# Blaizzy/mlx-audio

Hardware: AMD Instinct MI355X
Metric: audio samples/sec + real-time factor, Kokoro-82M TTS (higher is better)
Workload: dtype bf16 weights x fp32 activations: vocoder convs = fp16 hi pass (v_mfma_f32_32x32x16_f16) + block-scaled FP4 (e2m1) lo pass (v_mfma_scale_f32_32x32x64_f8f6f4 cbsz / blgp 4, OCP MX: E8M0 scale per row x 32 channels / per output column), fp32 accumulate; front end bf16 hi+lo split; 1 GPU; Kokoro-82M bf16 TTS, tokens->waveform, canonical short sentence T=80 F=264 (6.6 s @ 24 kHz); utterances_per_gpu=64, global_batch=64, samples_per_utterance=158400, parallelism=utterance-dp1, precision_mode=6, wire=fp32

## Files before the change

mlx_audio_amd/csrc/conv_common.h:

```cpp
#pragma once
#include <stdlib.h>
#include <type_traits>
#include "common.h"

namespace mi355conv {

__device__ __forceinline__ void glds16(const void* gsrc, void* ldst) {
  __builtin_amdgcn_global_load_lds((const __attribute__((address_space(1))) void*)gsrc,
                                   (__attribute__((address_space(3))) void*)ldst, 16, 0, 0);
}

__device__ __forceinline__ float gelu_erf(float x) { return 0.5f * x * (1.0f + erff(x * 0.70710678118654752f)); }
__device__ __forceinline__ float gelu_tanh(float x) { return 0.5f * x * (1.0f + tanhf(0.7978845608028654f * (x + 0.044715f * x * x * x))); }

template <int PREC>
__device__ __forceinline__ f32x16 mfma16(const bf16x8 a, const bf16x8 b, const f32x16 c) {
  if constexpr (PREC >= 3)
    return __builtin_amdgcn_mfma_f32_32x32x16_f16(__builtin_bit_cast(f16x8, a), __builtin_bit_cast(f16x8, b), c, 0, 0, 0);
  else
    return __builtin_amdgcn_mfma_f32_32x32x16_bf16(a, b, c, 0, 0, 0);
}
template <int PREC>
constexpr int a_images() { return (PREC == 2 || PREC == 4) ? 2 : 1; }
template <int PREC>
// ... 36 lines not shown
    const float sn = __builtin_amdgcn_sinf(k.al_rev * u);
    u = fmaf(k.ial, sn * sn, u);
  }
  return u;
}

__device__ __forceinline__ void lds_barrier() {
  asm volatile("s_waitcnt lgkmcnt(0)" ::: "memory");
  __builtin_amdgcn_s_barrier();
  asm volatile("" ::: "memory");
}

template <int MF, int NF, int WM, int WN, int EPI, bool EXT = false, int MT = MF, int MO = 0>
__device__ __forceinline__ void conv_epilogue(const mi355_conv_gemm_args& a, f32x16 (&acc)[MT][NF], const int b, const int l0,
                                              const int n0, const int wm, const int wn, const int lane, const int len_out,
                                              const bool folded) {
  const int len_up = a.lens_up ? a.lens_up[b] : a.up_Lout;
  const int len_up_c = len_up > 0 ? len_up : 1;
  float* yb = a.y + (int64_t)b * a.y_bstride;
  const float* rb = (a.res && !folded) ? a.res + (int64_t)b * a.res_bstride : nullptr;
  const bool accum = a.accumulate && !folded;
  const bool want_stats = a.stats_partial != nullptr;
  float sK[NF], s1[NF], s2[NF];
  int scnt[NF];
  const bool want_ext = EXT && a.ext_partial != nullptr;
#pragma unroll
  for (int nf = 0; nf < NF; ++nf) { sK[nf] = 0.f; s1[nf] = 0.f; s2[nf] = 0.f; scnt[nf] = 0; }
#pragma unroll
  for (int mf = 0; mf < MF; ++mf)
#pragma unroll
    for (int nf = 0; nf < NF; ++nf) {
      const int n = n0 + wn * WN + nf * 32 + (lane & 31);
      const bool nok = n < a.Cout;
      const int ncl = nok ? n : a.Cout - 1;
      int ocol = ncl, rph = 0;
      if (a.up_s) { rph = ncl / a.up_cout; ocol = ncl - rph * a.up_cout; }
      const float bias = a.bias ? a.bias[ocol] : 0.f;
      const float cscale = a.post_colscale ? a.post_colscale[ocol] : 1.f;
#pragma unroll
      for (int h = 0; h < 2; ++h) {
        int orows[8];
        bool ok[8];
        float rv[8];
#pragma unroll
        for (int q = 0; q < 8; ++q) {
          const int r = h * 8 + q;
// ... 225 lines not shown
          }
        }
#pragma unroll
        for (int q = 0; q < 8; ++q) {
          const int r = h * 8 + q;
          const float v = ((acc[mf][nf][r] + bias) + rv[q]) * oscale;
          *(float*)(yw + (yoff + (uint32_t)(mf * 32 + (r & 3) + 8 * (r >> 2)) * ystep)) = v;
        }
        __builtin_amdgcn_sched_barrier(0);
      }
  }
}

}

int mi355_conv_ws4_launch(const mi355_conv_gemm_args& a, hipStream_t st, int feat, int bn = 128);
bool mi355_conv_ws4_eligible(const mi355_conv_gemm_args& a, bool vec);
```

mlx_audio_amd/csrc/conv_gemm.hip:

```cpp
#include "conv_common.h"

using namespace mi355conv;

namespace {

constexpr int kThreads = 256;

struct split_geom {
  int ksplit, cpz;
  int lo_slices;
};

template <int BM, int BN, int PREC, bool VEC, bool SPLIT = false>
__global__ __launch_bounds__(kThreads) void conv_gemm_kernel(const mi355_conv_gemm_args a, const split_geom sg) {
  constexpr int WM = BM / 2, WN = BN / 2, MF = WM / 32, NF = WN / 32;
  constexpr int BBYTES = (BN / 32) * 2048;
  extern __shared__ __attribute__((aligned(16))) char smem[];

  const int tid = threadIdx.x, lane = tid & 63, wave = tid >> 6;
  const int wm = wave >> 1, wn = wave & 1;
  const int b = SPLIT ? (int)blockIdx.z / sg.ksplit : (int)blockIdx.z, l0 = blockIdx.x * BM, n0 = blockIdx.y * BN;
  const int len_out = a.lens_out ? a.lens_out[b] : a.Lout;
  if (l0 >= len_out) return;
  const int len_in = a.lens_in ? a.lens_in[b] : a.Lin;
// ... 548 lines not shown
    MI355_REQUIRE(a.stats_bstride % 2 == 0 && ((uintptr_t)a.stats_partial) % 8 == 0, "conv_gemm: stats_partial must be 8-byte aligned");
  }
  int tile = a.tile;
  t_mx_lo_slices = 0;
  if (a.y_split) {
    MI355_REQUIRE(a.y_split == 2 || a.y_split == 4, "conv_gemm: y_split must be 0, 2 (bfloat16 hi | lo) or 4 (IEEE half hi | lo)");
    MI355_REQUIRE(!a.accumulate, "conv_gemm: y_split cannot accumulate into y (y holds split words)");
    a.split_ws = nullptr;
  }
  if (a.x_split) {
    MI355_REQUIRE(a.x_split == a.precision && (a.precision == 2 || a.precision == 4), "conv_gemm: x_split must equal the launch's precision, 2 or 4");
    MI355_REQUIRE(a.pre_act == MI355_ACT_NONE && !a.pre_scale && !a.pre_fq, "conv_gemm: a split input takes no prologue");
    MI355_REQUIRE(!a.ext_partial && mi355_conv_ws4_eligible(a, vec), "conv_gemm: x_split needs 16-byte aligned channels-last rows and a window of <= 192 rows "
                  "(the wave-specialised kernel)");
    static const int ws_feat_x = getenv("MI355_CONV_WS_FEAT") ? atoi(getenv("MI355_CONV_WS_FEAT")) : 0;
    const int rc = a.Cout <= 64 ? mi355_conv_ws4_launch(a, st, ws_feat_x & 3, 64) : mi355_conv_ws4_launch(a, st, tile % 10000000 == 6128128 ? ((tile / 10000000) % 10) : ws_feat_x);
    return rc;
  }
  if (a.ext_partial) {
    MI355_REQUIRE(conv_ext_supported(a), "conv_gemm: ext_partial needs a launch mi355_conv_gemm_ext_supported accepts (pre_fq, precision 2, plain store, K > 1)");
    MI355_REQUIRE(a.ext_bstride % 2 == 0 && ((uintptr_t)a.ext_partial) % 8 == 0, "conv_gemm: ext_partial must be 8-byte aligned");
    static const int ws_feat_e = getenv("MI355_CONV_WS_FEAT") ? atoi(getenv("MI355_CONV_WS_FEAT")) : 0;
    return mi355_conv_ws4_launch(a, st, ws_feat_e & 3, a.Cout <= 64 ? 64 : 128);
  }
  if (a.precision == 5 || a.precision == 6) {
    static const long ws_min5 = getenv("MI355_CONV_WS_MIN_TILES") ? atol(getenv("MI355_CONV_WS_MIN_TILES")) : 128;
    static const bool no_ws5 = getenv("MI355_CONV_NO_WS") != nullptr;
    const long wgs128 = (long)a.B * ((a.Lout + 127) / 128) * ((a.Cout + 127) / 128);
    const bool want = tile % 10000000 == 6128128 || (tile == 0 && !no_ws5 && a.Cout > 64 && wgs128 >= ws_min5 && a.Cin >= 64);
    if (want && mi355_conv_ws4_eligible(a, vec)) {
      const int rc = mi355_conv_ws4_launch(a, st, tile == 0 ? 0 : (((tile / 10000000) % 10) | ((tile / 100000000) << 4)));
      if (rc != MI355_ERR_UNSUPPORTED) return rc;
    }
    MI355_REQUIRE(tile % 10000000 != 6128128, "conv_gemm: precisions 5 / 6 on the wave-specialised tile needs K = 3 (mod 4), a plain / LeakyReLU / Snake prologue, "
                  "no epilogue activation beyond LeakyReLU and 16-B aligned channels-last rows");
    t_mx_lo_slices = (a.K + 1) >> 1;
    a.precision = 4;
  }
  const bool mx_image = t_mx_lo_slices != 0;
  if (tile == 0) {
    const int bn = a.Cout <= 64 ? 64 : 128;
    const long wgs128 = (long)a.B * ((a.Lout + 127) / 128) * ((a.Cout + bn - 1) / bn);
    const int bm = (bn == 128 && wgs128 >= 512) ? 128 : 64;
    tile = bm * 1000 + bn;
    static const bool no_ws = getenv("MI355_CONV_NO_WS") != nullptr;
    static const int ws_feat = getenv("MI355_CONV_WS_FEAT") ? atoi(getenv("MI355_CONV_WS_FEAT")) : 0;
// ... 13 lines not shown
      const int ks = split_groups(wgs64, (a.Cin + 31) >> 5, a.K, (long)a.B * a.Lout, a.Cout, a.split_ws_bytes, 0);
      if (ks) return bn == 128 ? launch_split_p<64, 128>(a, st, ks) : launch_split_p<64, 64>(a, st, ks);
    }
  }
  if (tile % 10000000 == 2064128 || tile % 10000000 == 2064064) {
    MI355_REQUIRE(vec && a.split_ws, "conv_gemm: the split-K tiles need the 16-B aligned channels-last input path and a workspace (split_ws)");
    const bool wide = tile % 10000000 == 2064128;
    const long wgs64 = (long)a.B * ((a.Lout + 63) / 64) * ((a.Cout + (wide ? 127 : 63)) / (wide ? 128 : 64));
    const int ks = split_groups(wgs64, (a.Cin + 31) >> 5, a.K, (long)a.B * a.Lout, a.Cout, a.split_ws_bytes, tile / 10000000 ? tile / 10000000 : -1);
    MI355_REQUIRE(ks >= 2, "conv_gemm: nothing to split (C_in %d, K %d, workspace %lld bytes)", a.Cin, a.K, (long long)a.split_ws_bytes);
    return wide ? launch_split_p<64, 128>(a, st, ks) : launch_split_p<64, 64>(a, st, ks);
  }
  if (tile % 10000000 == 6128064) {
    MI355_REQUIRE(!mx_image, "conv_gemm: MX images (precision 5) have no 128 x 64 wave-specialised tile");
    MI355_REQUIRE(mi355_conv_ws4_eligible(a, vec), "conv_gemm: the wave-specialised tile needs 16-B aligned channels-last input rows and a window of <= 192 rows");
    return mi355_conv_ws4_launch(a, st, (tile / 10000000) & 11, 64);
  }
  if (tile % 10000000 == 6128128) {
    MI355_REQUIRE(mi355_conv_ws4_eligible(a, vec), "conv_gemm: the wave-specialised tile needs 16-B aligned channels-last input rows and a window of <= 192 rows");
    return mi355_conv_ws4_launch(a, st, ((tile / 10000000) % 10) | ((tile / 100000000) << 4));
  }
  if (a.stats_partial) {
    MI355_REQUIRE(vec, "conv_gemm: fused statistics need the 16-B aligned channels-last input path");
    tile = 128128;
  }
  if (!vec) {
    if (a.precision == 3) return launch<64, 64, 3, false>(a, st);
    if (a.precision == 4) return launch<64, 64, 4, false>(a, st);
    a.precision = 2;
    return launch<64, 64, 2, false>(a, st);
  }
  if (a.precision == 2) {
    switch (tile) {
      case 128128: return launch<128, 128, 2, true>(a, st);
      case 64128: return launch<64, 128, 2, true>(a, st);
// ... 25 lines not shown
```

mlx_audio_amd/csrc/conv_ws4.h:

```cpp
#pragma once
#include "conv_common.h"

namespace mi355conv {

extern int g_ws4_resident;

constexpr int kWs4Threads = 512;

enum { P_NONE = 0, P_LEAKY = 1, P_SNAKE = 2, P_SNAKEBETA = 3, P_ELU = 4 };

struct ws4_geom {
  int tiles_per_item, P, NT, glog, fold;
  int nch;
  int keff;
  int tap_rows;
  int R;
  int gemm;
  int nslices;
  int bn;
  int feat;
  int total_ids;
  unsigned long long* dbg;
};

constexpr int kDbgSlots = 48;

struct tile_t { int b, l0, n0, len_out, len_in; };

__device__ __forceinline__ bool decode_tile(const mi355_conv_gemm_args& a, const ws4_geom& q, const int id, tile_t& t) {
  const int kq = id >> 3;
  const int ny = kq % q.NT;
  const int pg = kq / q.NT;
  const int glog = q.glog;
  const int p = (((((pg >> glog) << 3) + (id & 7)) << glog)) | (pg & ((1 << glog) - 1));
  if (p >= q.P) return false;
  t.b = p / q.tiles_per_item;
  t.l0 = (p - t.b * q.tiles_per_item) * 128;
  t.n0 = ny * q.bn;
  t.len_out = a.lens_out ? a.lens_out[t.b] : a.Lout;
  if (t.l0 >= t.len_out) return false;
  t.len_in = a.lens_in ? a.lens_in[t.b] : a.Lin;
  return true;
}
__device__ __forceinline__ int next_work(const mi355_conv_gemm_args& a, const ws4_geom& q, int id, tile_t& t) {
  for (id += (int)gridDim.x; id < q.total_ids; id += (int)gridDim.x)
    if (decode_tile(a, q, id, t)) return id;
  return -1;
}

template <int PREC, int PRE, int EPI, bool GEMM, bool DBG = false, int ABL = 0, int BN = 128, bool FQ = false, bool CW = true>
__global__ __launch_bounds__(kWs4Threads, 4) void conv_ws4_kernel(const mi355_conv_gemm_args a, const ws4_geom q) {
  static_assert(!FQ || (!GEMM && (PRE == P_NONE || PRE == P_LEAKY || PRE == P_SNAKE)), "quantising prologues: conv mode, none / LeakyReLU / Snake");
  constexpr int BM = 128;
  static_assert(BN == 128 || BN == 64, "tile columns");
  constexpr bool MXP = PREC == 5 || PREC == 6;
  constexpr bool FP4 = PREC == 6;
// ... 14 lines not shown
  tile_t t0;
  int id0 = (int)blockIdx.x - (int)gridDim.x;
  id0 = next_work(a, q, id0, t0);
  if (id0 < 0) return;

  if (wave >= 4) {
    const int ptid = tid - 256;
    const int c4 = (ptid & 7) * 4;
    const int prow = ptid >> 3;
    const float* xbase = a.x + a.x_off;
    const int wrow0 = (wave - 4) * 8;
    constexpr int cstride = GEMM ? 64 : 32;
    float4 s0[NLD], s1[NLD];
    constexpr int NKC = 2 + ((PRE == P_SNAKE || PRE == P_SNAKEBETA) ? 1 : 0) + (PRE == P_SNAKEBETA ? 1 : 0);
    float4 k0[NKC], k1[NKC];
    struct item_t { int id, ci, b, l0, len_in; };
    auto advance = [&](item_t& it) {
      if (it.ci + 1 < nch) { ++it.ci; return; }
      tile_t t;
      it.id = next_work(a, q, it.id, t);
      it.ci = 0; it.b = t.b; it.l0 = t.l0; it.len_in = t.len_in;
    };

    constexpr bool FASTW = !FQ && (MXP || GEMM || PRE == P_NONE || PRE == P_LEAKY);
    const bool fastw_off = !MXP && (q.feat & 2);
    auto interior_window = [&](const item_t& it) {
      if (fastw_off) return false;
      if constexpr (GEMM) return it.l0 + 128 <= it.len_in && it.l0 + 128 <= a.Lin && it.ci * 64 + 64 <= a.Cin;
      const int r0 = it.l0 - a.pad;
      return r0 >= 0 && r0 + R <= it.len_in && r0 + R <= a.Lin && it.ci * 32 + 32 <= a.Cin;
    };
    auto loadA = [&](float4 (&areg)[NLD], float4 (&kreg)[NKC], const item_t& it) {
      const int chunk = it.ci, l0 = it.l0;
      const float* xb = xbase + (int64_t)it.b * a.x_bstride;
      {
        const int c = chunk * cstride + c4;
        const float* const safe = (const float*)a.w;
        const bool aff = !GEMM && a.pre_scale != nullptr;
        kreg[0] = *(const float4*)(aff ? a.pre_scale + (int64_t)it.b * a.pre_ld + c : safe);
        kreg[1] = *(const float4*)(aff ? a.pre_shift + (int64_t)it.b * a.pre_ld + c : safe);
        if constexpr (PRE == P_SNAKE || PRE == P_SNAKEBETA) kreg[2] = *(const float4*)(a.pre_alpha + c);
        if constexpr (PRE == P_SNAKEBETA) kreg[3] = *(const float4*)(a.pre_inv_beta + c);
      }
      if (FASTW && interior_window(it)) {
        const char* wb = (const char*)(xb + (int64_t)(GEMM ? l0 : l0 - a.pad) * a.ldx + chunk * cstride);
        const uint32_t loff = ((uint32_t)prow * (uint32_t)a.ldx + (uint32_t)c4) * 4u;
        const size_t pstep = (size_t)a.ldx * 128u;
#pragma unroll
        for (int i = 0; i < NLD; ++i) {
          const int ii = (GEMM || wrow0 + i * 32 < R) ? i : 0;
          if constexpr (GEMM) areg[i] = *(const float4*)(wb + (ii & 3) * pstep + (ii >> 2) * 128 + loff);
          else areg[i] = *(const float4*)(wb + ii * pstep + loff);
        }
        return;
      }
#pragma unroll
      for (int i = 0; i < NLD; ++i) {
        const int ii = (GEMM || wrow0 + i * 32 < R) ? i : 0;
        int gl = GEMM ? l0 + prow + 32 * (ii & 3) : l0 - a.pad + prow + 32 * ii;
        int c = chunk * cstride + (GEMM ? 32 * (ii >> 2) : 0) + c4;
        gl = gl < 0 ? 0 : (gl >= a.Lin ? a.Lin - 1 : gl);
        if (c >= a.Cin) c = 0;
        areg[i] = *(const float4*)(xb + (int64_t)gl * a.ldx + c);
      }
    };
    auto convertA_body = [&](const float4 (&areg)[NLD], const float4 (&kreg)[NKC], const item_t& it, char* A_hi, auto mask_tag) {
      constexpr bool MASK = decltype(mask_tag)::value;
      const int chunk = it.ci, l0 = it.l0, b = it.b, len_in = it.len_in;
      char* A_lo = A_hi + ABYTES;
      const int c = chunk * cstride + c4;
      float sc[4] = {1.f, 1.f, 1.f, 1.f}, sh[4] = {0.f, 0.f, 0.f, 0.f}, al[4] = {1.f, 1.f, 1.f, 1.f}, ial[4] = {1.f, 1.f, 1.f, 1.f};
      if constexpr (!GEMM) {
        const bool aff = a.pre_scale != nullptr;
// ... 17 lines not shown
          al[j] *= 0.15915494309189535f;
        }
      }
      const float slope = a.pre_slope;
      const FakeQuant fq = FQ ? FakeQuant(-a.pre_fq[2 * b], a.pre_fq[2 * b + 1]) : FakeQuant(0.f, 0.f);
      fq_coef fk[4];
      if constexpr (FQ) {
#pragma unroll
        for (int j = 0; j < 4; ++j)
          fk[j] = fq_load_coef(a.pre_scale, a.pre_shift, (int64_t)b * a.pre_ld, PRE == P_SNAKE ? MI355_ACT_SNAKE : MI355_ACT_NONE, a.pre_alpha, c + j);
      }
      const bool chan[4] = {c < a.Cin, c + 1 < a.Cin, c + 2 < a.Cin, c + 3 < a.Cin};
      const bool xs = PRE == P_NONE && NA == 2 && !FQ && !MXP && a.x_split != 0;
#pragma unroll
      for (int i = 0; i < NLD; ++i) {
        if (GEMM || wrow0 + i * 32 < R) {
          const int r = prow + i * 32;
          if (GEMM || r < R) {
            const int gl = GEMM ? l0 + prow + 32 * (i & 3) : l0 - a.pad + r;
            const bool rowok = gl >= 0 && gl < len_in;
            const int cb = c + (GEMM ? 32 * (i >> 2) : 0);
            const float v[4] = {areg[i].x, areg[i].y, areg[i].z, areg[i].w};
            if constexpr (PRE == P_NONE && NA == 2 && !FQ && !MXP) {
              if (xs) {
                uint32_t w[4];
#pragma unroll
                for (int j = 0; j < 4; ++j) w[j] = (!MASK || (rowok && (cb + j) < a.Cin)) ? __builtin_bit_cast(uint32_t, v[j]) : 0u;
                const int xaddr = r * 64 + ((((c4 >> 3) ^ ((r >> 2) & 3))) << 4) + ((c4 & 4) << 1);
                uint2 xh, xl;
                xh.x = __builtin_amdgcn_perm(w[1], w[0], 0x05040100u);
                xh.y = __builtin_amdgcn_perm(w[3], w[2], 0x05040100u);
// ... 114 lines not shown
              if ((ptid & 7) == 0) *(uint8_t*)(A_l8 + R * LP + r) = (uint8_t)sb;
            }
          }
        }
      }
    };

    auto convertA = [&](const float4 (&areg)[NLD], const float4 (&kreg)[NKC], const item_t& it, char* A_hi) {
      if constexpr (FASTW) {
        if (interior_window(it)) { convertA_body(areg, kreg, it, A_hi, std::false_type{}); return; }
      }
      convertA_body(areg, kreg, it, A_hi, std::true_type{});
    };


    item_t ia{id0, 0, t0.b, t0.l0, t0.len_in};
    item_t ib = ia;
    advance(ib);
    constexpr bool work = (ABL & 4) == 0;
    unsigned long long* pdbg = nullptr;
    unsigned long long pc_conv = 0, pc_bar = 0, pc_load = 0, pc_items = 0, pc_first = 0, pc_t = 0;
    if constexpr (DBG && MXP) {
      if (wave == 4 && (blockIdx.x & 15) == 0 && q.dbg) pdbg = q.dbg + (size_t)(blockIdx.x >> 4) * kDbgSlots;
      if (pdbg) pc_first = pc_t = __builtin_amdgcn_s_memtime();
    }
    auto pstamp = [&](unsigned long long& acc_c) {
      if constexpr (DBG && MXP) {
        if (pdbg) { const unsigned long long n = __builtin_amdgcn_s_memtime(); acc_c += n - pc_t; pc_t = n; }
      }
    };
    if (work) loadA(s0, k0, ia);
// ... 40 lines not shown
  if (!(q.feat & 1)) __builtin_amdgcn_s_setprio(1);
  const int NTp = ((a.Cout + 127) >> 7) << 2;
  const int64_t wstep = (int64_t)NTp * 2048;
  const int nsteps = nch * keff;
  const int last_slice = q.nslices - 1;
  const int fold = q.fold;
  unsigned long long* dbg = nullptr;
  if constexpr (DBG) {
    if (wave == 0 && (blockIdx.x & 15) == 0 && q.dbg) dbg = q.dbg + (size_t)(blockIdx.x >> 4) * kDbgSlots;
  }
  int jbuf = 0;
  int ntile = 0;
  tile_t t = t0;
  for (int id = id0; id >= 0; id = next_work(a, q, id, t), ++ntile) {
    const int b = t.b, l0 = t.l0, n0 = t.n0, len_out = t.len_out;
    int lane = lane_k;
    asm volatile("" : "+v"(lane));
    const int hl = lane & 31, hh = lane >> 5;
    if constexpr (DBG) {
      if (dbg && lane == 0 && ntile < 8) dbg[4 * ntile] = __builtin_amdgcn_s_memtime();
      if (dbg && lane == 0 && (ntile == 0 || ntile == 7)) dbg[32 + (ntile == 7)] = wall_clock64();
    }
    const char* wfrag = (const char*)a.w + ((int64_t)((n0 >> 5) + wn * NF)) * 2048 + lane * 16;
    auto wptr = [&](const int s) { return wfrag + (int64_t)(s < last_slice ? s : last_slice) * wstep; };
    bf16x8 b0[NB], b1[NB];
    if constexpr (!MXP) {
#pragma unroll
      for (int f = 0; f < NB; ++f) b0[f] = *(const bf16x8*)(wfrag + f * 1024);
    }

// ... 25 lines not shown
#pragma unroll
            for (int r = 0; r < 16; ++r) rv[r] = *(const float*)(rw + (roff + (uint32_t)(mf * 32 + (r & 3) + 8 * (r >> 2)) * rpb + (uint32_t)(nf * 128)));
          }
          if (a.accumulate) {
#pragma unroll
            for (int r = 0; r < 16; ++r) rv[r] += *(const float*)(yr + (yoff + (uint32_t)(mf * 32 + (r & 3) + 8 * (r >> 2)) * ypb + (uint32_t)(nf * 128)));
          }
#pragma unroll
          for (int r = 0; r < 16; ++r) acc[mf][nf][r] = rv[r];
        }
    } else if ((ABL & 8) == 0 && fold) {
#pragma unroll
      for (int mf = 0; mf < MF; ++mf)
#pragma unroll
        for (int nf = 0; nf < NF; ++nf) {
          const int n = n0 + wn * WN + nf * 32 + hl;
          const bool nok = n < a.Cout;
          const int ncl = nok ? n : a.Cout - 1;
#pragma unroll
          for (int h = 0; h < 2; ++h) {
            float rv[8];
            int us[8];
#pragma unroll
            for (int qq = 0; qq < 8; ++qq) {
              const int r = h * 8 + qq;
              us[qq] = l0 + wm * WM + mf * 32 + (r & 3) + 8 * (r >> 2) + 4 * hh;
              rv[qq] = 0.f;
            }
            if (rb) {
#pragma unroll
// ... 25 lines not shown
        if constexpr ((ABL & 1) != 0) {
          if (!first) { asm volatile("" : "+v"(w) : "s"(src)); return; }
        }
        const i32x4 lo4 = *(const i32x4*)(src + wlane);
        if (FP4 && lo_item) {
          w = __builtin_shufflevector(lo4, lo4, 0, 1, 2, 3, 4, 5, 6, 7);
          return;
        }
        const i32x4 hi4 = *(const i32x4*)(src + 1024 + wlane);
        w = __builtin_shufflevector(lo4, hi4, 0, 1, 2, 3, 4, 5, 6, 7);
      };
      i32x8 w0, w1;
      ldW(w0, 0, true);
      if constexpr ((ABL & 1) != 0) w1 = w0;
      i32x8 qv[4];
      int sv[4] = {0, 0, 0, 0};
#pragma unroll
      for (int g = 0; g < 4; ++g)
#pragma unroll
        for (int e = 0; e < 8; ++e) qv[g][e] = 0;
      int hlx = hl, hhx = hh;
      int lbH = 0, lbL = 0, lbS = 0;
      auto fresh = [&]() {
        asm volatile("" : "+v"(hlx), "+v"(hhx));
        lbH = hlx * HP + hhx * 16;
        if constexpr (FP4) {
          lbL = (hlx + hhx * dil) * LP;
          lbS = hlx + hhx * dil;
        } else {
          lbL = hlx * LP + hhx * 16;
          lbS = hlx;
// ... 9 lines not shown
        i32x4 v0, v1;
        if constexpr ((ABL & 2) != 0) { v0 = (i32x4){la, la, la, la}; v1 = v0; }
        else {
          v0 = *(const i32x4*)(Abase + (la + uoff));
          v1 = *(const i32x4*)(Abase + (la + uoff) + 32 * HP);
        }
        qv[g] = __builtin_shufflevector(v0, v1, 0, 1, 2, 3, 4, 5, 6, 7);
      };
      auto rdL = [&](const int mf, const int p) {
        const int t1 = 2 * p + 1 < K ? 2 * p + 1 : K - 1;
        const int u0 = mf * 32 + 2 * p * dil, u1 = mf * 32 + t1 * dil;
        const int ubase = jbuf * WBYTES + ABYTES;
        int la = lbL, ls = lbS;
        asm volatile("" : "+v"(la), "+v"(ls));
        i32x4 x0, x1;
        int sc;
        if constexpr (FP4) {
          const int back = (2 * p + 1 < K) ? 0 : dil;
          if (back) { la -= hhx * back * LP; ls -= hhx * back; }
          x0 = *(const i32x4*)(Abase + (la + (ubase + u0 * LP)));
          x1 = x0;
          sc = (int)*(const uint8_t*)(Abase + (ls + (ubase + R * LP + u0)));
        } else if constexpr ((ABL & 2) != 0) {
          x0 = (i32x4){la, la, la, la}; x1 = x0; sc = 120 + (ls & 7);
        } else {
          x0 = *(const i32x4*)(Abase + (la + (ubase + u0 * LP)));
          x1 = *(const i32x4*)(Abase + (la + (ubase + u1 * LP)));
          sc = (int)*(const uint8_t*)(Abase + (ls + (ubase + R * LP + (hhx ? u1 : u0))));
        }
        qv[mf] = __builtin_shufflevector(x0, x1, 0, 1, 2, 3, 4, 5, 6, 7);
        sv[mf] = sc;
      };
      auto mmH = [&](const int g, const i32x8& w) {
        const int kk = g >> 1, m0 = 2 * (g & 1);
        const bf16x8 bfrag = kk ? hi4(w) : lo4(w);
        acc[m0][0] = mfma16<PREC>(lo4(qv[g]), bfrag, acc[m0][0]);
        acc[m0 + 1][0] = mfma16<PREC>(hi4(qv[g]), bfrag, acc[m0 + 1][0]);
      };
      auto mmL = [&](const int mf, const i32x8& w) {
        if constexpr (FP4) {
          const i32x4 a4 = __builtin_shufflevector(qv[mf], qv[mf], 0, 1, 2, 3), b4 = __builtin_shufflevector(w, w, 0, 1, 2, 3);
          asm volatile("s_nop 1\n\tv_mfma_scale_f32_32x32x64_f8f6f4 %0, %1, %2, %0, %3, %4 op_sel_hi:[0,0,0] cbsz:4 blgp:4" : "+v"(acc[mf][0]) : "v"(a4), "v"(b4), "v"(sv[mf]), "v"(bsc));
        } else {
          asm volatile("s_nop 1\n\tv_mfma_scale_f32_32x32x64_f8f6f4 %0, %1, %2, %0, %3, %4 op_sel_hi:[0,0,0]" : "+v"(acc[mf][0]) : "v"(qv[mf]), "v"(w), "v"(sv[mf]), "v"(bsc));
        }
      };
      auto hi_tap = [&](const int tp, const i32x8& w, auto last) {
        constexpr bool LAST = decltype(last)::value;
        fresh();
#pragma unroll
        for (int g = 0; g < 4; ++g) {
          mmH(g, w);
          if constexpr (LAST) rdL(g, 0);
          else rdH(g, tp + 1);
          __builtin_amdgcn_sched_barrier(0);
        }
      };
      auto lo_pair = [&](const int p, const i32x8& w, const bool more) {
        fresh();
// ... 136 lines not shown
        i32x4 x0, x1;
        int sc;
        if constexpr ((ABL & 2) != 0) {
          x0 = (i32x4){la, la, la, la}; x1 = x0; sc = 120 + (ls & 7);
        } else {
          x0 = *(const i32x4*)(Abase + (la + (ubase + u0 * LP)));
          x1 = *(const i32x4*)(Abase + (la + (ubase + u1 * LP)));
          sc = (int)*(const uint8_t*)(Abase + (ls + (ubase + R * LP + (hhx ? u1 : u0))));
        }
        if (mf == 0) { qa = __builtin_shufflevector(x0, x1, 0, 1, 2, 3, 4, 5, 6, 7); sa = sc; }
        else { qb = __builtin_shufflevector(x0, x1, 0, 1, 2, 3, 4, 5, 6, 7); sb2 = sc; }
      };
      auto mmH = [&](const int g, const i32x8 (&w)[2]) {
        const int kk = g >> 1, mf = g & 1;
        const bf16x8 h = g == 0 ? lo4(qa) : (g == 1 ? hi4(qa) : (g == 2 ? lo4(qb) : hi4(qb)));
#pragma unroll
        for (int nf = 0; nf < NF; ++nf) acc[mf][nf] = mfma16<PREC>(h, kk ? hi4(w[nf]) : lo4(w[nf]), acc[mf][nf]);
      };
      auto mmL = [&](const int mf, const i32x8 (&w)[2]) {
        if (mf == 0) {
          asm volatile("s_nop 1\n\tv_mfma_scale_f32_32x32x64_f8f6f4 %0, %1, %2, %0, %3, %4 op_sel_hi:[0,0,0]" : "+v"(acc[0][0]) : "v"(qa), "v"(w[0]), "v"(sa), "v"(bsc));
          asm volatile("v_mfma_scale_f32_32x32x64_f8f6f4 %0, %1, %2, %0, %3, %4 op_sel:[0,1,0] op_sel_hi:[0,0,0]" : "+v"(acc[0][1]) : "v"(qa), "v"(w[1]), "v"(sa), "v"(bsc));
        } else {
          asm volatile("s_nop 1\n\tv_mfma_scale_f32_32x32x64_f8f6f4 %0, %1, %2, %0, %3, %4 op_sel_hi:[0,0,0]" : "+v"(acc[1][0]) : "v"(qb), "v"(w[0]), "v"(sb2), "v"(bsc));
          asm volatile("v_mfma_scale_f32_32x32x64_f8f6f4 %0, %1, %2, %0, %3, %4 op_sel:[0,1,0] op_sel_hi:[0,0,0]" : "+v"(acc[1][1]) : "v"(qb), "v"(w[1]), "v"(sb2), "v"(bsc));
        }
      };
      auto hi_tap = [&](const int tp, const i32x8 (&w)[2], auto last) {
        constexpr bool LAST = decltype(last)::value;
        fresh();
        mmH(0, w);
        if constexpr (!LAST) rdH(0, tp + 1);
        __builtin_amdgcn_sched_barrier(0);
        mmH(1, w);
// ... 79 lines not shown
      auto rdA = [&](bf16x8& h, bf16x8& l, const int g, const int tp) {
        const int kk = g >> 1, mf = g & 1;
        const int row = wm * WM + mf * 32 + hl + tp * q.tap_rows;
        const int cidx = kk * 2 + hh;
        const int addr = row * 64 + ((cidx ^ ((row >> 2) & 3)) << 4);
        const char* A_hi = Abase + jbuf * WBYTES;
        if constexpr ((ABL & 2) != 0) {
          asm volatile("" : "+v"(h), "+v"(l) : "v"(addr));
        } else {
          h = *(const bf16x8*)(A_hi + addr);
          if constexpr (NA == 2) l = *(const bf16x8*)(A_hi + ABYTES + addr);
        }
      };
      auto mm = [&](const bf16x8& h, const bf16x8& l, const int g, const bf16x8 (&bf)[NB]) {
        const int kk = g >> 1, mf = g & 1;
#pragma unroll
        for (int nf = 0; nf < NF; ++nf) acc[mf][nf] = mfma16<PREC>(h, bf[2 * nf + kk], acc[mf][nf]);
        if constexpr (NA == 2) {
#pragma unroll
          for (int nf = 0; nf < NF; ++nf) acc[mf][nf] = mfma16<PREC>(l, bf[2 * nf + kk], acc[mf][nf]);
        }
      };
      auto tap_body = [&](const bf16x8 (&bf)[NB], const bool first) {
        if (tap == 0) {
          lds_barrier();
          if constexpr (DBG) {
            if (first && dbg && lane == 0 && ntile < 8) dbg[4 * ntile + 1] = __builtin_amdgcn_s_memtime();
          }
          rdA(ah0, al0, 0, 0);
        }
// ... 45 lines not shown
#pragma unroll
      for (int mf = 0; mf < MF; ++mf)
#pragma unroll
        for (int nf = 0; nf < NF; ++nf)
#pragma unroll
          for (int r = 0; r < 16; ++r) tsum += acc[mf][nf][r];
      if (tsum == 1.2345e-30f) yb[0] = tsum;
      continue;
    }
    const bool plain = a.up_s == 0 && a.post_act == MI355_ACT_NONE && (fold || (!a.res && !a.accumulate)) && !a.post_colscale && !a.y_split;
    if constexpr (COLW) {
      if (plain && interior) {
        conv_epilogue_interior<2, NF, 64, WN, FQ, MF, 0>(a, acc, b, l0, n0, 0, wn, lane);
        conv_epilogue_interior<2, NF, 64, WN, FQ, MF, 2>(a, acc, b, l0, n0, 1, wn, lane);
      } else {
        conv_epilogue<2, NF, 64, WN, EPI, FQ, MF, 0>(a, acc, b, l0, n0, 0, wn, lane, len_out, fold != 0);
        conv_epilogue<2, NF, 64, WN, EPI, FQ, MF, 2>(a, acc, b, l0, n0, 1, wn, lane, len_out, fold != 0);
      }
    } else {
      bool up_interior = false;
      if constexpr (EPI == 0 && !FQ && BN == 128 && PRE == P_LEAKY && !GEMM) {
        if (a.up_s != 0 && interior && a.post_act == MI355_ACT_NONE && !a.accumulate && !a.post_colscale && !a.y_split && !a.stats_partial && a.res_shift == 0 &&
            (a.up_cout & 31) == 0) {
          const int len_up = a.lens_up ? a.lens_up[b] : a.up_Lout;
          up_interior = (int64_t)l0 * a.up_s - a.up_p >= 0 && (int64_t)(l0 + BM - 1) * a.up_s + (a.up_s - 1) - a.up_p < len_up;
        }
      }
      if (plain && interior) conv_epilogue_interior<MF, NF, WM, WN, FQ>(a, acc, b, l0, n0, wm, wn, lane);
      else if (up_interior) conv_epilogue_up_interior<MF, NF, WM, WN>(a, acc, b, l0, n0, wm, wn, lane);
      else conv_epilogue<MF, NF, WM, WN, EPI, FQ>(a, acc, b, l0, n0, wm, wn, lane, len_out, fold != 0);
    }
    if constexpr (DBG) {
      if (dbg && lane == 0 && ntile < 8) dbg[4 * ntile + 3] = __builtin_amdgcn_s_memtime();
    }
  }
  if (!(q.feat & 1)) __builtin_amdgcn_s_setprio(0);
}

inline bool gemm_mode(const mi355_conv_gemm_args& a) { return a.K == 1 && a.Cin >= 64 && a.pre_act == MI355_ACT_NONE && !a.pre_scale && !a.pre_fq; }

template <int PREC, int PRE, int EPI, bool GEMM, bool DBG = false, int ABL = 0, int BN = 128, bool FQ = false, bool CW = true>
int launch_ws4(const mi355_conv_gemm_args& a, hipStream_t st, const int feat, unsigned long long* dbg = nullptr) {
  ws4_geom q;
  q.bn = BN;
  q.gemm = GEMM ? 1 : 0;
// ... 50 lines not shown
inline int pre_kind(const mi355_conv_gemm_args& a) {
  switch (a.pre_act) {
    case MI355_ACT_NONE: return P_NONE;
    case MI355_ACT_LEAKY: return P_LEAKY;
    case MI355_ACT_SNAKE: return a.pre_inv_beta ? P_SNAKEBETA : P_SNAKE;
    case MI355_ACT_ELU: return P_ELU;
  }
  return -1;
}

#define WS4_CASE(PREC, PRE, EPI) \
  if (bn == 128 && pre == PRE && epi == EPI && !gemm) return launch_ws4<PREC, PRE, EPI, false>(a, st, feat)
#define WS4_GEMM(PREC, EPI) \
  if (bn == 128 && epi == EPI && gemm) return launch_ws4<PREC, P_NONE, EPI, true>(a, st, feat)
#define WS4_CASE_N64(PREC, PRE, EPI) \
  if (bn == 64 && pre == PRE && epi == EPI && !gemm) return launch_ws4<PREC, PRE, EPI, false, false, 0, 64>(a, st, feat & 15)
#define WS4_GEMM_N64(PREC, EPI) \
  if (bn == 64 && epi == EPI && gemm) return launch_ws4<PREC, P_NONE, EPI, true, false, 0, 64>(a, st, feat & 15)

}

int mi355_conv_ws4_p2(const mi355_conv_gemm_args& a, hipStream_t st, int feat, unsigned long long* dbg, int bn);
int mi355_conv_ws4_p4(const mi355_conv_gemm_args& a, hipStream_t st, int feat, int bn);
int mi355_conv_ws4_p13(const mi355_conv_gemm_args& a, hipStream_t st, int feat, int bn);
int mi355_conv_ws4_fq(const mi355_conv_gemm_args& a, hipStream_t st, int feat, int bn);
int mi355_conv_ws4_p5(const mi355_conv_gemm_args& a, hipStream_t st, int feat, int bn);
int mi355_conv_ws4_p6(const mi355_conv_gemm_args& a, hipStream_t st, int feat, int bn);
int mi355_conv_ws4_p5_probe(const mi355_conv_gemm_args& a, hipStream_t st, int feat, unsigned long long* dbg);
```

mlx_audio_amd/csrc/conv_ws4.hip:

```cpp
#include "conv_ws4.h"

using namespace mi355conv;

namespace {
unsigned long long* g_dbg_buffer = nullptr;
}

namespace mi355conv {
int g_ws4_resident = 0;
}

extern "C" int mi355_conv_ws4_resident(int wgs) {
  MI355_REQUIRE(wgs >= 0, "conv_ws4_resident: negative count");
  mi355conv::g_ws4_resident = wgs;
  return MI355_OK;
}

bool mi355_conv_ws4_eligible(const mi355_conv_gemm_args& a, bool vec) {
  if (!vec || a.Lin <= 0 || a.flat_valid != 0) return false;
  if (a.precision == 5 || a.precision == 6)
    return a.K % 4 == 3 && 128 + (a.K - 1) * a.dil <= 192 && a.Cout > 64 && !a.pre_fq && (pre_kind(a) == P_NONE || pre_kind(a) == P_LEAKY || pre_kind(a) == P_SNAKE) &&
           epi_family(a) == 0;
  if (!gemm_mode(a) && 128 + (a.K - 1) * a.dil > 192) return false;
  return a.precision >= 1 && a.precision <= 4 && pre_kind(a) >= 0;
}

extern "C" int mi355_conv_ws4_debug_buffer(void* p) {
  g_dbg_buffer = (unsigned long long*)p;
  return MI355_OK;
}

int mi355_conv_ws4_p2(const mi355_conv_gemm_args& a, hipStream_t st, int feat, unsigned long long* dbg, int bn) {
  const int pre = pre_kind(a), epi = epi_family(a);
  const bool gemm = gemm_mode(a);
  if (bn == 128 && (feat & 4) && pre == P_SNAKE && epi == 0 && !gemm) return launch_ws4<2, P_SNAKE, 0, false, true>(a, st, feat, dbg);
  if (const int abl = bn == 128 ? feat >> 4 : 0) {
    if (gemm && epi == 0) {
      switch (abl) {
        case 1: return launch_ws4<2, P_NONE, 0, true, false, 1>(a, st, feat & 15);
        case 4: return launch_ws4<2, P_NONE, 0, true, false, 4>(a, st, feat & 15);
        case 5: return launch_ws4<2, P_NONE, 0, true, false, 5>(a, st, feat & 15);
      }
    }
    MI355_REQUIRE(pre == P_SNAKE && epi == 0 && !gemm, "conv_gemm(ws4): ablation tiles exist for the precision-2 Snake kernel and the plain GEMM mode only");
    switch (abl) {
      case 1: return launch_ws4<2, P_SNAKE, 0, false, false, 1>(a, st, feat & 15);
      case 2: return launch_ws4<2, P_SNAKE, 0, false, false, 2>(a, st, feat & 15);
      case 3: return launch_ws4<2, P_SNAKE, 0, false, false, 3>(a, st, feat & 15);
      case 4: return launch_ws4<2, P_SNAKE, 0, false, false, 4>(a, st, feat & 15);
      case 7: return launch_ws4<2, P_SNAKE, 0, false, false, 7>(a, st, feat & 15);
    }
// ... 8 lines not shown
  WS4_CASE(2, P_NONE, 1);
  WS4_GEMM(2, 0);
  WS4_GEMM(2, 1);
  WS4_GEMM(2, 2);
  WS4_GEMM(2, 3);
  WS4_CASE_N64(2, P_NONE, 0);
  WS4_CASE_N64(2, P_LEAKY, 0);
  WS4_CASE_N64(2, P_SNAKE, 0);
  WS4_CASE_N64(2, P_ELU, 0);
  WS4_GEMM_N64(2, 0);
  return MI355_ERR_UNSUPPORTED;
}

int mi355_conv_ws4_launch(const mi355_conv_gemm_args& a, hipStream_t st, int feat, int bn) {
  int rc = MI355_ERR_UNSUPPORTED;
  if (a.pre_fq) rc = a.precision == 2 ? mi355_conv_ws4_fq(a, st, feat & 3, bn) : MI355_ERR_UNSUPPORTED;
  else if (a.precision == 2) rc = mi355_conv_ws4_p2(a, st, feat, g_dbg_buffer, bn);
  else if (a.precision == 4) rc = mi355_conv_ws4_p4(a, st, feat & 3, bn);
  else if (a.precision == 6) rc = (feat & ~9) ? mi355_conv_ws4_p5_probe(a, st, feat, g_dbg_buffer) : mi355_conv_ws4_p6(a, st, feat & 9, bn);
  else if (a.precision == 5) rc = (feat & ~11) ? mi355_conv_ws4_p5_probe(a, st, feat, g_dbg_buffer) : mi355_conv_ws4_p5(a, st, feat & 11, bn);
  else if (a.precision == 1 || a.precision == 3) rc = mi355_conv_ws4_p13(a, st, feat & 3, bn);
  if (rc == MI355_ERR_UNSUPPORTED)
    mi355_set_error("conv_gemm(ws4): no instantiation for precision %d, prologue %d, epilogue family %d, %d-column tiles", a.precision, pre_kind(a), epi_family(a), bn);
  return rc;
}
```

mlx_audio_amd/csrc/conv_ws4_p5.hip:

```cpp
#include "conv_ws4.h"

using namespace mi355conv;

int mi355_conv_ws4_p5(const mi355_conv_gemm_args& a, hipStream_t st, int feat, int bn) {
  const int pre = pre_kind(a), epi = epi_family(a);
  const bool gemm = false;
  if ((feat & 2) && pre == P_SNAKE && epi == 0) return launch_ws4<5, P_SNAKE, 0, false, false, 0, 128, false, false>(a, st, feat & 9);
  WS4_CASE(5, P_NONE, 0);
  WS4_CASE(5, P_LEAKY, 0);
  WS4_CASE(5, P_SNAKE, 0);
  return MI355_ERR_UNSUPPORTED;
}
```

Before: 201.6 million samples/s.

## Skip dead 32-row blocks in tail tiles of wave-specialised conv kernel

Each tile now records how many of its four 32-row M blocks hold valid output rows, clamped by the sequence and upsampled lengths. The producer skips loads, the consumer skips the hi and lo MFMAs and epilogue stores for dead blocks, and fully dead waves only take part in the barriers. This removes wasted compute and memory traffic on partial tiles at the end of each utterance. Feature bit 128 turns the skip off, and the extra predicates and asm register pins add some branch and scheduling cost.

Result: slower. 197.8 million samples/s (-1.8%).

```diff
diff --git a/mlx_audio_amd/csrc/conv_common.h b/mlx_audio_amd/csrc/conv_common.h
--- a/mlx_audio_amd/csrc/conv_common.h
+++ b/mlx_audio_amd/csrc/conv_common.h
@@ -74,7 +74,7 @@
 template <int MF, int NF, int WM, int WN, int EPI, bool EXT = false, int MT = MF, int MO = 0>
 __device__ __forceinline__ void conv_epilogue(const mi355_conv_gemm_args& a, f32x16 (&acc)[MT][NF], const int b, const int l0,
                                               const int n0, const int wm, const int wn, const int lane, const int len_out,
-                                              const bool folded) {
+                                              const bool folded, const int mf_live = MF) {
   const int len_up = a.lens_up ? a.lens_up[b] : a.up_Lout;
   const int len_up_c = len_up > 0 ? len_up : 1;
   float* yb = a.y + (int64_t)b * a.y_bstride;
@@ -90,6 +90,7 @@
   for (int mf = 0; mf < MF; ++mf)
 #pragma unroll
     for (int nf = 0; nf < NF; ++nf) {
+      if (mf >= mf_live) continue;
       const int n = n0 + wn * WN + nf * 32 + (lane & 31);
       const bool nok = n < a.Cout;
       const int ncl = nok ? n : a.Cout - 1;
@@ -345,5 +346,7 @@
 
 }
 
+constexpr int kWs4FeatNoTailSkip = 128;
+inline int mi355_conv_ws4_tile_feat(const int tile) { return ((tile / 10000000) % 10) | ((tile / 100000000) << 4); }
 int mi355_conv_ws4_launch(const mi355_conv_gemm_args& a, hipStream_t st, int feat, int bn = 128);
 bool mi355_conv_ws4_eligible(const mi355_conv_gemm_args& a, bool vec);
diff --git a/mlx_audio_amd/csrc/conv_gemm.hip b/mlx_audio_amd/csrc/conv_gemm.hip
--- a/mlx_audio_amd/csrc/conv_gemm.hip
+++ b/mlx_audio_amd/csrc/conv_gemm.hip
@@ -586,7 +586,7 @@
     MI355_REQUIRE(!a.ext_partial && mi355_conv_ws4_eligible(a, vec), "conv_gemm: x_split needs 16-byte aligned channels-last rows and a window of <= 192 rows "
                   "(the wave-specialised kernel)");
     static const int ws_feat_x = getenv("MI355_CONV_WS_FEAT") ? atoi(getenv("MI355_CONV_WS_FEAT")) : 0;
-    const int rc = a.Cout <= 64 ? mi355_conv_ws4_launch(a, st, ws_feat_x & 3, 64) : mi355_conv_ws4_launch(a, st, tile % 10000000 == 6128128 ? ((tile / 10000000) % 10) : ws_feat_x);
+    const int rc = a.Cout <= 64 ? mi355_conv_ws4_launch(a, st, ws_feat_x & 3, 64) : mi355_conv_ws4_launch(a, st, tile % 10000000 == 6128128 ? (mi355_conv_ws4_tile_feat(tile) & (15 | kWs4FeatNoTailSkip)) : ws_feat_x);
     return rc;
   }
   if (a.ext_partial) {
@@ -601,7 +601,7 @@
     const long wgs128 = (long)a.B * ((a.Lout + 127) / 128) * ((a.Cout + 127) / 128);
     const bool want = tile % 10000000 == 6128128 || (tile == 0 && !no_ws5 && a.Cout > 64 && wgs128 >= ws_min5 && a.Cin >= 64);
     if (want && mi355_conv_ws4_eligible(a, vec)) {
-      const int rc = mi355_conv_ws4_launch(a, st, tile == 0 ? 0 : (((tile / 10000000) % 10) | ((tile / 100000000) << 4)));
+      const int rc = mi355_conv_ws4_launch(a, st, tile == 0 ? 0 : mi355_conv_ws4_tile_feat(tile));
       if (rc != MI355_ERR_UNSUPPORTED) return rc;
     }
     MI355_REQUIRE(tile % 10000000 != 6128128, "conv_gemm: precisions 5 / 6 on the wave-specialised tile needs K = 3 (mod 4), a plain / LeakyReLU / Snake prologue, "
@@ -645,11 +645,11 @@
   if (tile % 10000000 == 6128064) {
     MI355_REQUIRE(!mx_image, "conv_gemm: MX images (precision 5) have no 128 x 64 wave-specialised tile");
     MI355_REQUIRE(mi355_conv_ws4_eligible(a, vec), "conv_gemm: the wave-specialised tile needs 16-B aligned channels-last input rows and a window of <= 192 rows");
-    return mi355_conv_ws4_launch(a, st, (tile / 10000000) & 11, 64);
+    return mi355_conv_ws4_launch(a, st, mi355_conv_ws4_tile_feat(tile) & (11 | kWs4FeatNoTailSkip), 64);
   }
   if (tile % 10000000 == 6128128) {
     MI355_REQUIRE(mi355_conv_ws4_eligible(a, vec), "conv_gemm: the wave-specialised tile needs 16-B aligned channels-last input rows and a window of <= 192 rows");
-    return mi355_conv_ws4_launch(a, st, ((tile / 10000000) % 10) | ((tile / 100000000) << 4));
+    return mi355_conv_ws4_launch(a, st, mi355_conv_ws4_tile_feat(tile));
   }
   if (a.stats_partial) {
     MI355_REQUIRE(vec, "conv_gemm: fused statistics need the 16-B aligned channels-last input path");
diff --git a/mlx_audio_amd/csrc/conv_ws4.h b/mlx_audio_amd/csrc/conv_ws4.h
--- a/mlx_audio_amd/csrc/conv_ws4.h
+++ b/mlx_audio_amd/csrc/conv_ws4.h
@@ -25,7 +25,19 @@
 
 constexpr int kDbgSlots = 48;
 
-struct tile_t { int b, l0, n0, len_out, len_in; };
+struct tile_t { int b, l0, n0, len_out, len_in, mb; };
+
+__device__ __forceinline__ int tile_live_blocks(const mi355_conv_gemm_args& a, const ws4_geom& q, const tile_t& t) {
+  if (q.feat & kWs4FeatNoTailSkip) return 4;
+  int len = t.len_out;
+  if (a.up_s) {
+    const int len_up = a.lens_up ? a.lens_up[t.b] : a.up_Lout;
+    const int lu = (len_up + a.up_p + a.up_s - 1) / a.up_s;
+    len = lu < len ? lu : len;
+  }
+  const int mb = (len - t.l0 + 31) >> 5;
+  return mb < 1 ? 1 : (mb > 4 ? 4 : mb);
+}
 
 __device__ __forceinline__ bool decode_tile(const mi355_conv_gemm_args& a, const ws4_geom& q, const int id, tile_t& t) {
   const int kq = id >> 3;
@@ -40,6 +52,7 @@
   t.len_out = a.lens_out ? a.lens_out[t.b] : a.Lout;
   if (t.l0 >= t.len_out) return false;
   t.len_in = a.lens_in ? a.lens_in[t.b] : a.Lin;
+  t.mb = tile_live_blocks(a, q, t);
   return true;
 }
 __device__ __forceinline__ int next_work(const mi355_conv_gemm_args& a, const ws4_geom& q, int id, tile_t& t) {
@@ -84,12 +97,16 @@
     float4 s0[NLD], s1[NLD];
     constexpr int NKC = 2 + ((PRE == P_SNAKE || PRE == P_SNAKEBETA) ? 1 : 0) + (PRE == P_SNAKEBETA ? 1 : 0);
     float4 k0[NKC], k1[NKC];
-    struct item_t { int id, ci, b, l0, len_in; };
+    struct item_t { int id, ci, b, l0, len_in, mb; };
     auto advance = [&](item_t& it) {
       if (it.ci + 1 < nch) { ++it.ci; return; }
       tile_t t;
       it.id = next_work(a, q, it.id, t);
-      it.ci = 0; it.b = t.b; it.l0 = t.l0; it.len_in = t.len_in;
+      it.ci = 0; it.b = t.b; it.l0 = t.l0; it.len_in = t.len_in; it.mb = t.mb;
+    };
+    auto pass_live = [&](const int i, const item_t& it) {
+      if constexpr (GEMM) return (i & 3) < it.mb;
+      else return wrow0 + i * 32 < R - 32 * (4 - it.mb);
     };
 
     constexpr bool FASTW = !FQ && (MXP || GEMM || PRE == P_NONE || PRE == P_LEAKY);
@@ -118,7 +135,7 @@
         const size_t pstep = (size_t)a.ldx * 128u;
 #pragma unroll
         for (int i = 0; i < NLD; ++i) {
-          const int ii = (GEMM || wrow0 + i * 32 < R) ? i : 0;
+          const int ii = pass_live(i, it) ? i : 0;
           if constexpr (GEMM) areg[i] = *(const float4*)(wb + (ii & 3) * pstep + (ii >> 2) * 128 + loff);
           else areg[i] = *(const float4*)(wb + ii * pstep + loff);
         }
@@ -126,7 +143,7 @@
       }
 #pragma unroll
       for (int i = 0; i < NLD; ++i) {
-        const int ii = (GEMM || wrow0 + i * 32 < R) ? i : 0;
+        const int ii = pass_live(i, it) ? i : 0;
         int gl = GEMM ? l0 + prow + 32 * (ii & 3) : l0 - a.pad + prow + 32 * ii;
         int c = chunk * cstride + (GEMM ? 32 * (ii >> 2) : 0) + c4;
         gl = gl < 0 ? 0 : (gl >= a.Lin ? a.Lin - 1 : gl);
@@ -174,7 +191,7 @@
       const bool xs = PRE == P_NONE && NA == 2 && !FQ && !MXP && a.x_split != 0;
 #pragma unroll
       for (int i = 0; i < NLD; ++i) {
-        if (GEMM || wrow0 + i * 32 < R) {
+        if (pass_live(i, it)) {
           const int r = prow + i * 32;
           if (GEMM || r < R) {
             const int gl = GEMM ? l0 + prow + 32 * (i & 3) : l0 - a.pad + r;
@@ -319,7 +336,7 @@
     };
 
 
-    item_t ia{id0, 0, t0.b, t0.l0, t0.len_in};
+    item_t ia{id0, 0, t0.b, t0.l0, t0.len_in, t0.mb};
     item_t ib = ia;
     advance(ib);
     constexpr bool work = (ABL & 4) == 0;
@@ -390,6 +407,15 @@
   tile_t t = t0;
   for (int id = id0; id >= 0; id = next_work(a, q, id, t), ++ntile) {
     const int b = t.b, l0 = t.l0, n0 = t.n0, len_out = t.len_out;
+    const int mb = t.mb;
+    const int nlive = COLW ? mb : (mb - wm * MF < 0 ? 0 : (mb - wm * MF > MF ? MF : mb - wm * MF));
+    if constexpr (!COLW) {
+      if (nlive == 0) {
+        for (int c = 0; c < nch; ++c) lds_barrier();
+        jbuf ^= nch & 1;
+        continue;
+      }
+    }
     int lane = lane_k;
     asm volatile("" : "+v"(lane));
     const int hl = lane & 31, hh = lane >> 5;
@@ -445,6 +471,7 @@
       for (int mf = 0; mf < MF; ++mf)
 #pragma unroll
         for (int nf = 0; nf < NF; ++nf) {
+          if (mf >= nlive) continue;
           const int n = n0 + wn * WN + nf * 32 + hl;
           const bool nok = n < a.Cout;
           const int ncl = nok ? n : a.Cout - 1;
@@ -500,7 +527,7 @@
       ldW(w0, 0, true);
       if constexpr ((ABL & 1) != 0) w1 = w0;
       i32x8 qv[4];
-      int sv[4] = {0, 0, 0, 0};
+      uint8_t sv[4] = {0, 0, 0, 0};
 #pragma unroll
       for (int g = 0; g < 4; ++g)
 #pragma unroll
@@ -540,35 +567,44 @@
         int la = lbL, ls = lbS;
         asm volatile("" : "+v"(la), "+v"(ls));
         i32x4 x0, x1;
-        int sc;
+        uint8_t sc;
         if constexpr (FP4) {
           const int back = (2 * p + 1 < K) ? 0 : dil;
           if (back) { la -= hhx * back * LP; ls -= hhx * back; }
           x0 = *(const i32x4*)(Abase + (la + (ubase + u0 * LP)));
           x1 = x0;
-          sc = (int)*(const uint8_t*)(Abase + (ls + (ubase + R * LP + u0)));
+          sc = *(const uint8_t*)(Abase + (ls + (ubase + R * LP + u0)));
         } else if constexpr ((ABL & 2) != 0) {
           x0 = (i32x4){la, la, la, la}; x1 = x0; sc = 120 + (ls & 7);
         } else {
           x0 = *(const i32x4*)(Abase + (la + (ubase + u0 * LP)));
           x1 = *(const i32x4*)(Abase + (la + (ubase + u1 * LP)));
-          sc = (int)*(const uint8_t*)(Abase + (ls + (ubase + R * LP + (hhx ? u1 : u0))));
+          sc = *(const uint8_t*)(Abase + (ls + (ubase + R * LP + (hhx ? u1 : u0))));
         }
         qv[mf] = __builtin_shufflevector(x0, x1, 0, 1, 2, 3, 4, 5, 6, 7);
-        sv[mf] = sc;
+        sv[mf] = (uint8_t)sc;
       };
       auto mmH = [&](const int g, const i32x8& w) {
         const int kk = g >> 1, m0 = 2 * (g & 1);
         const bf16x8 bfrag = kk ? hi4(w) : lo4(w);
-        acc[m0][0] = mfma16<PREC>(lo4(qv[g]), bfrag, acc[m0][0]);
-        acc[m0 + 1][0] = mfma16<PREC>(hi4(qv[g]), bfrag, acc[m0 + 1][0]);
+        const bf16x8 a0 = lo4(qv[g]), a1 = hi4(qv[g]);
+        asm volatile("" ::"v"(a0));
+        if (m0 == 0 || m0 < mb) acc[m0][0] = mfma16<PREC>(a0, bfrag, acc[m0][0]);
+        asm volatile("" ::"v"(a1));
+        if (m0 + 1 < mb) acc[m0 + 1][0] = mfma16<PREC>(a1, bfrag, acc[m0 + 1][0]);
       };
       auto mmL = [&](const int mf, const i32x8& w) {
+        const bool dead = mf > 0 && mf >= mb;
+        const int sca = (int)sv[mf];
         if constexpr (FP4) {
           const i32x4 a4 = __builtin_shufflevector(qv[mf], qv[mf], 0, 1, 2, 3), b4 = __builtin_shufflevector(w, w, 0, 1, 2, 3);
-          asm volatile("s_nop 1\n\tv_mfma_scale_f32_32x32x64_f8f6f4 %0, %1, %2, %0, %3, %4 op_sel_hi:[0,0,0] cbsz:4 blgp:4" : "+v"(acc[mf][0]) : "v"(a4), "v"(b4), "v"(sv[mf]), "v"(bsc));
+          asm volatile("" ::"v"(a4), "v"(sca));
+          if (dead) return;
+          asm volatile("s_nop 1\n\tv_mfma_scale_f32_32x32x64_f8f6f4 %0, %1, %2, %0, %3, %4 op_sel_hi:[0,0,0] cbsz:4 blgp:4" : "+v"(acc[mf][0]) : "v"(a4), "v"(b4), "v"(sca), "v"(bsc));
         } else {
-          asm volatile("s_nop 1\n\tv_mfma_scale_f32_32x32x64_f8f6f4 %0, %1, %2, %0, %3, %4 op_sel_hi:[0,0,0]" : "+v"(acc[mf][0]) : "v"(qv[mf]), "v"(w), "v"(sv[mf]), "v"(bsc));
+          asm volatile("" ::"v"(qv[mf]), "v"(sca));
+          if (dead) return;
+          asm volatile("s_nop 1\n\tv_mfma_scale_f32_32x32x64_f8f6f4 %0, %1, %2, %0, %3, %4 op_sel_hi:[0,0,0]" : "+v"(acc[mf][0]) : "v"(qv[mf]), "v"(w), "v"(sca), "v"(bsc));
         }
       };
       auto hi_tap = [&](const int tp, const i32x8& w, auto last) {
@@ -735,10 +771,15 @@
       auto mmH = [&](const int g, const i32x8 (&w)[2]) {
         const int kk = g >> 1, mf = g & 1;
         const bf16x8 h = g == 0 ? lo4(qa) : (g == 1 ? hi4(qa) : (g == 2 ? lo4(qb) : hi4(qb)));
+        asm volatile("" ::"v"(h));
+        if (mf > 0 && mf >= nlive) return;
 #pragma unroll
         for (int nf = 0; nf < NF; ++nf) acc[mf][nf] = mfma16<PREC>(h, kk ? hi4(w[nf]) : lo4(w[nf]), acc[mf][nf]);
       };
       auto mmL = [&](const int mf, const i32x8 (&w)[2]) {
+        if (mf == 0) asm volatile("" ::"v"(qa), "v"(sa));
+        else asm volatile("" ::"v"(qb), "v"(sb2));
+        if (mf > 0 && mf >= nlive) return;
         if (mf == 0) {
           asm volatile("s_nop 1\n\tv_mfma_scale_f32_32x32x64_f8f6f4 %0, %1, %2, %0, %3, %4 op_sel_hi:[0,0,0]" : "+v"(acc[0][0]) : "v"(qa), "v"(w[0]), "v"(sa), "v"(bsc));
           asm volatile("v_mfma_scale_f32_32x32x64_f8f6f4 %0, %1, %2, %0, %3, %4 op_sel:[0,1,0] op_sel_hi:[0,0,0]" : "+v"(acc[0][1]) : "v"(qa), "v"(w[1]), "v"(sa), "v"(bsc));
@@ -848,6 +889,9 @@
       };
       auto mm = [&](const bf16x8& h, const bf16x8& l, const int g, const bf16x8 (&bf)[NB]) {
         const int kk = g >> 1, mf = g & 1;
+        if constexpr (NA == 2) asm volatile("" ::"v"(h), "v"(l));
+        else asm volatile("" ::"v"(h));
+        if (mf > 0 && mf >= nlive) return;
 #pragma unroll
         for (int nf = 0; nf < NF; ++nf) acc[mf][nf] = mfma16<PREC>(h, bf[2 * nf + kk], acc[mf][nf]);
         if constexpr (NA == 2) {
@@ -923,8 +967,8 @@
         conv_epilogue_interior<2, NF, 64, WN, FQ, MF, 0>(a, acc, b, l0, n0, 0, wn, lane);
         conv_epilogue_interior<2, NF, 64, WN, FQ, MF, 2>(a, acc, b, l0, n0, 1, wn, lane);
       } else {
-        conv_epilogue<2, NF, 64, WN, EPI, FQ, MF, 0>(a, acc, b, l0, n0, 0, wn, lane, len_out, fold != 0);
-        conv_epilogue<2, NF, 64, WN, EPI, FQ, MF, 2>(a, acc, b, l0, n0, 1, wn, lane, len_out, fold != 0);
+        conv_epilogue<2, NF, 64, WN, EPI, FQ, MF, 0>(a, acc, b, l0, n0, 0, wn, lane, len_out, fold != 0, mb);
+        if (mb > 2) conv_epilogue<2, NF, 64, WN, EPI, FQ, MF, 2>(a, acc, b, l0, n0, 1, wn, lane, len_out, fold != 0, mb - 2);
       }
     } else {
       bool up_interior = false;
@@ -937,7 +981,7 @@
       }
       if (plain && interior) conv_epilogue_interior<MF, NF, WM, WN, FQ>(a, acc, b, l0, n0, wm, wn, lane);
       else if (up_interior) conv_epilogue_up_interior<MF, NF, WM, WN>(a, acc, b, l0, n0, wm, wn, lane);
-      else conv_epilogue<MF, NF, WM, WN, EPI, FQ>(a, acc, b, l0, n0, wm, wn, lane, len_out, fold != 0);
+      else conv_epilogue<MF, NF, WM, WN, EPI, FQ>(a, acc, b, l0, n0, wm, wn, lane, len_out, fold != 0, nlive);
     }
     if constexpr (DBG) {
       if (dbg && lane == 0 && ntile < 8) dbg[4 * ntile + 3] = __builtin_amdgcn_s_memtime();
@@ -1018,9 +1062,9 @@
 #define WS4_GEMM(PREC, EPI) \
   if (bn == 128 && epi == EPI && gemm) return launch_ws4<PREC, P_NONE, EPI, true>(a, st, feat)
 #define WS4_CASE_N64(PREC, PRE, EPI) \
-  if (bn == 64 && pre == PRE && epi == EPI && !gemm) return launch_ws4<PREC, PRE, EPI, false, false, 0, 64>(a, st, feat & 15)
+  if (bn == 64 && pre == PRE && epi == EPI && !gemm) return launch_ws4<PREC, PRE, EPI, false, false, 0, 64>(a, st, feat & (15 | kWs4FeatNoTailSkip))
 #define WS4_GEMM_N64(PREC, EPI) \
-  if (bn == 64 && epi == EPI && gemm) return launch_ws4<PREC, P_NONE, EPI, true, false, 0, 64>(a, st, feat & 15)
+  if (bn == 64 && epi == EPI && gemm) return launch_ws4<PREC, P_NONE, EPI, true, false, 0, 64>(a, st, feat & (15 | kWs4FeatNoTailSkip))
 
 }
 
diff --git a/mlx_audio_amd/csrc/conv_ws4.hip b/mlx_audio_amd/csrc/conv_ws4.hip
--- a/mlx_audio_amd/csrc/conv_ws4.hip
+++ b/mlx_audio_amd/csrc/conv_ws4.hip
@@ -34,7 +34,7 @@
   const int pre = pre_kind(a), epi = epi_family(a);
   const bool gemm = gemm_mode(a);
   if (bn == 128 && (feat & 4) && pre == P_SNAKE && epi == 0 && !gemm) return launch_ws4<2, P_SNAKE, 0, false, true>(a, st, feat, dbg);
-  if (const int abl = bn == 128 ? feat >> 4 : 0) {
+  if (const int abl = bn == 128 ? (feat >> 4) & 7 : 0) {
     if (gemm && epi == 0) {
       switch (abl) {
         case 1: return launch_ws4<2, P_NONE, 0, true, false, 1>(a, st, feat & 15);
@@ -73,12 +73,12 @@
 
 int mi355_conv_ws4_launch(const mi355_conv_gemm_args& a, hipStream_t st, int feat, int bn) {
   int rc = MI355_ERR_UNSUPPORTED;
-  if (a.pre_fq) rc = a.precision == 2 ? mi355_conv_ws4_fq(a, st, feat & 3, bn) : MI355_ERR_UNSUPPORTED;
+  if (a.pre_fq) rc = a.precision == 2 ? mi355_conv_ws4_fq(a, st, feat & (3 | kWs4FeatNoTailSkip), bn) : MI355_ERR_UNSUPPORTED;
   else if (a.precision == 2) rc = mi355_conv_ws4_p2(a, st, feat, g_dbg_buffer, bn);
-  else if (a.precision == 4) rc = mi355_conv_ws4_p4(a, st, feat & 3, bn);
-  else if (a.precision == 6) rc = (feat & ~9) ? mi355_conv_ws4_p5_probe(a, st, feat, g_dbg_buffer) : mi355_conv_ws4_p6(a, st, feat & 9, bn);
-  else if (a.precision == 5) rc = (feat & ~11) ? mi355_conv_ws4_p5_probe(a, st, feat, g_dbg_buffer) : mi355_conv_ws4_p5(a, st, feat & 11, bn);
-  else if (a.precision == 1 || a.precision == 3) rc = mi355_conv_ws4_p13(a, st, feat & 3, bn);
+  else if (a.precision == 4) rc = mi355_conv_ws4_p4(a, st, feat & (3 | kWs4FeatNoTailSkip), bn);
+  else if (a.precision == 6) rc = (feat & ~(9 | kWs4FeatNoTailSkip)) ? mi355_conv_ws4_p5_probe(a, st, feat, g_dbg_buffer) : mi355_conv_ws4_p6(a, st, feat, bn);
+  else if (a.precision == 5) rc = (feat & ~(11 | kWs4FeatNoTailSkip)) ? mi355_conv_ws4_p5_probe(a, st, feat, g_dbg_buffer) : mi355_conv_ws4_p5(a, st, feat, bn);
+  else if (a.precision == 1 || a.precision == 3) rc = mi355_conv_ws4_p13(a, st, feat & (3 | kWs4FeatNoTailSkip), bn);
   if (rc == MI355_ERR_UNSUPPORTED)
     mi355_set_error("conv_gemm(ws4): no instantiation for precision %d, prologue %d, epilogue family %d, %d-column tiles", a.precision, pre_kind(a), epi_family(a), bn);
   return rc;
diff --git a/mlx_audio_amd/csrc/conv_ws4_p5.hip b/mlx_audio_amd/csrc/conv_ws4_p5.hip
--- a/mlx_audio_amd/csrc/conv_ws4_p5.hip
+++ b/mlx_audio_amd/csrc/conv_ws4_p5.hip
@@ -5,7 +5,7 @@
 int mi355_conv_ws4_p5(const mi355_conv_gemm_args& a, hipStream_t st, int feat, int bn) {
   const int pre = pre_kind(a), epi = epi_family(a);
   const bool gemm = false;
-  if ((feat & 2) && pre == P_SNAKE && epi == 0) return launch_ws4<5, P_SNAKE, 0, false, false, 0, 128, false, false>(a, st, feat & 9);
+  if ((feat & 2) && pre == P_SNAKE && epi == 0) return launch_ws4<5, P_SNAKE, 0, false, false, 0, 128, false, false>(a, st, feat & (9 | kWs4FeatNoTailSkip));
   WS4_CASE(5, P_NONE, 0);
   WS4_CASE(5, P_LEAKY, 0);
   WS4_CASE(5, P_SNAKE, 0);
```
